# real-stanford/semantic-abstraction

Hardware: AMD Instinct MI355X
Metric: scenes/sec (relevancy+3D-UNet infer), 480x480x16-label x128^3 (higher is better)
Workload: dtype f16 (MFMA operands, fp32 accumulate; UNet hi/lo-split = fp32-equivalent); 1 GPU; end-to-end relevancy->fusion->OVSSC per scene: 480x480 RGB-D, 16 labels, ViT-B/16, 'ours' saliency config (2448 tile forwards), 128^3 voxels, 80000 input points; scene-sharded; arch=ViT-B/16, unet_precision=exact, tile_chunk_streams=1, scenes_per_gpu=26, parallelism=scene-shard x1, mode=throughput

## Files before the change

### semantic-abstraction_amd/csrc/gemm.hip

```cpp
#include "semabs_common.h"
#include <hip/hip_ext.h>
#include <type_traits>
#include <mutex>

#define BK 64
enum { EPI_BIAS_F16 = 0, EPI_BIAS_GELU_F16 = 1, EPI_BIAS_RESID_F32 = 2, EPI_BIAS_F32 = 3, EPI_ROWMAP_ADD_F32 = 4, EPI_MULROW_F16 = 5 };

struct GemmArgs {
    const f16* A; const f16* B; void* C; const float* bias; const float* addend;
    long M; int N, K; long lda; int ldb; long ldc;
    int g_in, g_out, g_off;
    int n_tiles_n; int n_tiles_m; int group_m; int n_blocks;
    int sc_w;
    int reverse;
    f16* ln_xg; const float* ln_gamma; float* ln_part;
    const float* ln_center;
    const float* ln_rowac; const float* ln_colsum;
    f16* lo_out; int lo_cols; long ld_lo;
#ifdef SEMABS_TUNING
    int ablate;
    unsigned long long* trace;
    unsigned long long* ptrace; int ptrace_wg;
#endif
};
#ifdef SEMABS_TUNING
#define GEMM_ABL(bit) ((g.ablate & (bit)) != 0)
#else
#define GEMM_ABL(bit) (false)
#endif

template <int BKT>
__device__ __forceinline__ int swz_off(int row, int chunk) {
    if (BKT == 64) return row * 128 + ((chunk ^ ((row >> 1) & 7)) << 4);
    return row * 64 + ((chunk ^ ((row >> 2) & 3)) << 4);
}

template <int N> __device__ __forceinline__ void wait_vmcnt() { asm volatile("s_waitcnt vmcnt(%0)" ::"n"(N) : "memory"); }

template <int EPI, int BM, int BN, int BKT, int WGM, int WGN, int STAGES>
__global__ __launch_bounds__(64 * WGM * WGN, ((BM / WGM) * (BN / WGN) <= 64 * 64 && WGM * WGN >= 8) ? 4 : 2) void k_gemm_f16(GemmArgs g) {
    constexpr int NW = WGM * WGN;
    constexpr int WTM = BM / WGM, WTN = BN / WGN, TM = WTM / 32, TN = WTN / 32;
    constexpr int ROWB = BKT * 2;
    constexpr int RPP = 1024 / ROWB;
    constexpr int CPR = ROWB / 16;
    constexpr int A_BYTES = BM * ROWB, BUF = (BM + BN) * ROWB;
    constexpr int PPW = (BM + BN) / RPP / NW;
    static_assert((BM + BN) / RPP % NW == 0 && WTN == 64 && WTM % 32 == 0 && STAGES >= 2, "tile / wave layout");
    static_assert(STAGES * BUF >= NW * 8192, "epilogue staging needs 8 KB per wave");
    extern __shared__ __attribute__((aligned(16))) char smem[];
    const int tid = threadIdx.x, lane = tid & 63;
    const int wid = __builtin_amdgcn_readfirstlane(tid >> 6);
    const int wm = wid / WGN, wn = wid % WGN;

    int b = blockIdx.x;
    {
        const int nb = g.n_blocks, q = nb >> 3, r = nb & 7, xcd = b & 7, k = b >> 3;
        b = (xcd < r ? xcd * (q + 1) : r * (q + 1) + (xcd - r) * q) + k;
    }
    int tm, tn;
    {
        const int per_group = g.group_m * g.n_tiles_n, gid = b / per_group, first_m = gid * g.group_m;
        const int gsz = (g.n_tiles_m - first_m < g.group_m) ? g.n_tiles_m - first_m : g.group_m;
        const int r = b - gid * per_group;
        tm = first_m + r % gsz; tn = r / gsz;
    }
    const long m0 = (long)tm * BM;
    const int n0 = tn * BN;

    const f16* src[PPW];
// ... 70 lines not shown
    __builtin_amdgcn_s_barrier();

    if (GEMM_ABL(8) && acc[0][0][0] != 12345.678f) return;
    float* st = reinterpret_cast<float*>(smem + wid * 8192);
    const int cchunk = lane & 15;
    const int ncol = n0 + wn * WTN + cchunk * 4;
    float4 bv = make_float4(0.f, 0.f, 0.f, 0.f);
    if (g.bias) bv = *reinterpret_cast<const float4*>(g.bias + ncol);
#pragma unroll
    for (int i = 0; i < TM; ++i) {
#pragma unroll
        for (int j = 0; j < 2; ++j)
#pragma unroll
            for (int r = 0; r < 16; ++r) {
                int row = (r & 3) + 8 * (r >> 2) + 4 * (lane >> 5);
                st[row * 64 + j * 32 + (lane & 31)] = acc[i][j][r];
            }
        __builtin_amdgcn_s_waitcnt(0xc07f);
        __builtin_amdgcn_wave_barrier();
        if (EPI == EPI_BIAS_F16 || EPI == EPI_BIAS_GELU_F16) {
            const int c8 = lane & 7;
            const int ncol8 = n0 + wn * WTN + c8 * 8;
            float4 b0 = make_float4(0.f, 0.f, 0.f, 0.f), b1 = b0;
            if (g.bias) { b0 = *reinterpret_cast<const float4*>(g.bias + ncol8); b1 = *reinterpret_cast<const float4*>(g.bias + ncol8 + 4); }
#pragma unroll
            for (int it = 0; it < 4; ++it) {
                const int row = it * 8 + (lane >> 3);
                const long m = m0 + wm * WTM + i * 32 + row;
                if (m >= g.M) continue;
                const float4 v0 = *reinterpret_cast<const float4*>(st + row * 64 + c8 * 8);
                const float4 v1 = *reinterpret_cast<const float4*>(st + row * 64 + c8 * 8 + 4);
                float v[8] = {v0.x + b0.x, v0.y + b0.y, v0.z + b0.z, v0.w + b0.w, v1.x + b1.x, v1.y + b1.y, v1.z + b1.z, v1.w + b1.w};
                f16x8 h;
#pragma unroll
                for (int e = 0; e < 8; ++e) {
                    if (EPI == EPI_BIAS_GELU_F16) v[e] = v[e] * __builtin_amdgcn_rcpf(1.f + __expf(-1.702f * v[e]));
                    h[e] = (f16)v[e];
                }
                if (GEMM_ABL(16) && v[0] != 12345.678f) continue;
                *reinterpret_cast<f16x8*>(reinterpret_cast<f16*>(g.C) + m * g.ldc + ncol8) = h;
            }
        } else {
#pragma unroll 4
        for (int it = 0; it < 8; ++it) {
            int row = it * 4 + (lane >> 4);
            long m = m0 + wm * WTM + i * 32 + row;
            if (m >= g.M) continue;
            float4 v = *reinterpret_cast<const float4*>(st + row * 64 + cchunk * 4);
            v.x += bv.x; v.y += bv.y; v.z += bv.z; v.w += bv.w;
            if (GEMM_ABL(16) && v.x != 12345.678f) continue;
            if (EPI == EPI_BIAS_RESID_F32) {
                float4* p = reinterpret_cast<float4*>(reinterpret_cast<float*>(g.C) + m * g.ldc + ncol);
                float4 o = *p;
                o.x += v.x; o.y += v.y; o.z += v.z; o.w += v.w;
                *p = o;
            } else if (EPI == EPI_BIAS_F32) {
                *reinterpret_cast<float4*>(reinterpret_cast<float*>(g.C) + m * g.ldc + ncol) = v;
            } else {
                long grp = m / g.g_in; int within = (int)(m - grp * g.g_in);
                long orow = grp * g.g_out + g.g_off + within;
                if (g.addend) {
                    float4 a = *reinterpret_cast<const float4*>(g.addend + (long)(g.g_off + within) * g.N + ncol);
                    v.x += a.x; v.y += a.y; v.z += a.z; v.w += a.w;
                }
                *reinterpret_cast<float4*>(reinterpret_cast<float*>(g.C) + orow * g.ldc + ncol) = v;
            }
        }
        }
        __builtin_amdgcn_wave_barrier();
    }
}
// ... 193 lines not shown
            __builtin_amdgcn_sched_barrier(0);
            asm volatile("s_nop 7\n\ts_nop 7" ::: "memory");
            __builtin_amdgcn_sched_barrier(0);
        };
        constexpr int ROWB = OUT16 ? 64 : 128;
        constexpr int LPR = ROWB / 16;
        constexpr int RPI = 64 / LPR;
        constexpr int NIT = 64 / RPI;
        constexpr int PASSB = 64 * ROWB;
        char* const ep = smem + wid * 16384;
        float bia[2][8];
#pragma unroll
        for (int hb = 0; hb < 2; ++hb) {
            const int ncol = n0 + hb * 128 + wc * 32 + kg * 8;
#pragma unroll
            for (int e = 0; e < 8; ++e) bia[hb][e] = 0.f;
            if (g.bias) {
                const float4 b0 = *reinterpret_cast<const float4*>(g.bias + ncol), b1 = *reinterpret_cast<const float4*>(g.bias + ncol + 4);
                bia[hb][0] = b0.x; bia[hb][1] = b0.y; bia[hb][2] = b0.z; bia[hb][3] = b0.w; bia[hb][4] = b1.x; bia[hb][5] = b1.y; bia[hb][6] = b1.z; bia[hb][7] = b1.w;
            }
        }
        const int wswz = OUT16 ? ((l15 >> 1) & 3) : (l15 & 7);
        auto lds_write = [&](int pass) {
            const int hb = pass >> 1, ha = pass & 1;
            char* buf = ep + (pass & 1) * PASSB;
            f32x4 w[4][OUT16 ? 1 : 2];
#pragma unroll
            for (int i = 0; i < 4; ++i) {
                float v[8];
#pragma unroll
                for (int e = 0; e < 4; ++e) { v[e] = acc[ha][i][hb][0][e] + bia[hb][e]; v[4 + e] = acc[ha][i][hb][1][e] + bia[hb][4 + e]; }
                if constexpr (OUT16) {
                    f16x8 h;
#pragma unroll
                    for (int e = 0; e < 8; ++e) {
                        if (EPI == EPI_BIAS_GELU_F16) v[e] = v[e] * __builtin_amdgcn_rcpf(1.f + __expf(-1.702f * v[e]));
                        h[e] = (f16)v[e];
                    }
                    w[i][0] = __builtin_bit_cast(f32x4, h);
                } else {
                    w[i][0] = f32x4{v[0], v[1], v[2], v[3]};
                    w[i][OUT16 ? 0 : 1] = f32x4{v[4], v[5], v[6], v[7]};
                }
            }
            __builtin_amdgcn_sched_barrier(0);
#pragma unroll
            for (int i = 0; i < 4; ++i) {
                char* row = buf + (i * 16 + l15) * ROWB;
                if constexpr (OUT16) {
                    *reinterpret_cast<f32x4*>(row + ((kg ^ wswz) << 4)) = w[i][0];
                } else {
                    *reinterpret_cast<f32x4*>(row + (((2 * kg) ^ wswz) << 4)) = w[i][0];
                    *reinterpret_cast<f32x4*>(row + (((2 * kg + 1) ^ wswz) << 4)) = w[i][OUT16 ? 0 : 1];
                }
            }
            __builtin_amdgcn_sched_barrier(0);
        };
        const int crow = lane / LPR, cchunk = lane % LPR;
        auto lds_read = [&](int pass, int it) {
            const int row = it * RPI + crow;
            const int rswz = OUT16 ? ((row >> 1) & 3) : (row & 7);
            return *reinterpret_cast<const f32x4*>(ep + (pass & 1) * PASSB + row * ROWB + ((cchunk ^ rswz) << 4));
        };
        const long mw = m0 + wr * 64;
        const unsigned ldcb = (unsigned)g.ldc * ES;
        if constexpr (EPI == EPI_ROWMAP_ADD_F32) {
            const long grp0 = mw / g.g_in; const long orow0 = grp0 * g.g_out + g.g_off + (mw - grp0 * g.g_in);
            const long mlast = g.M - 1; const long grpl = mlast / g.g_in; const long orowl = grpl * g.g_out + g.g_off + (mlast - grpl * g.g_in);
            const __amdgpu_buffer_rsrc_t rC = gemm_rsrc(reinterpret_cast<const float*>(g.C) + orow0 * g.ldc + (n0 + wc * 32),
                                                        (orowl - orow0) * (long)ldcb + (long)(g.N - n0 - wc * 32) * ES);
#pragma unroll
// ... 502 lines not shown
        if (wid == 0 || wid == 4) {
            const int nst = g.K / 64 * 16;
            for (int i = lane; i < nst && i < 1024; i += 64)
                g.ptrace[(wid >> 2) * 1024 + i] = *reinterpret_cast<unsigned long long*>(smem + 2 * BUFSZ + (wid >> 2) * 8192 + i * 8);
        }
    }
#endif
#ifdef SEMABS_TUNING
    if (g.trace) {
        asm volatile("s_waitcnt vmcnt(0)" ::: "memory");
        const unsigned long long t_end = __builtin_amdgcn_s_memrealtime();
        if (tid == 0) {
            unsigned hw, xcc;
            asm volatile("s_getreg_b32 %0, hwreg(HW_REG_HW_ID)" : "=s"(hw));
            asm volatile("s_getreg_b32 %0, hwreg(HW_REG_XCC_ID)" : "=s"(xcc));
            unsigned long long* tr = g.trace + (size_t)vb * 8;
            tr[0] = t_start; tr[1] = t_main; tr[2] = t_end; tr[3] = ((unsigned long long)xcc << 32) | hw; tr[4] = c_start; tr[5] = c_main;
        }
    }
#endif
    if (PERS) {
        __builtin_amdgcn_s_waitcnt(0xc07f);
        __builtin_amdgcn_s_barrier();
    }
    vb += (int)gridDim.x;
    } while (PERS && vb < g.n_blocks);
#undef GABL
#undef GEMM8_SYNC
#undef GEMM8_END
#undef GEMM8_INTERLEAVE
#undef GEMM8_STAMP
}

template <int EPI, bool LNC = false, bool QKLO = false>
__global__ __launch_bounds__(512) void k_gemm8p(GemmArgs g) {
    static_assert(!QKLO || EPI == EPI_BIAS_F16, "the low halves exist for the plain fp16 output only");
    static_assert(EPI == EPI_BIAS_F16 || EPI == EPI_BIAS_GELU_F16 || EPI == EPI_BIAS_RESID_F32, "fp16-output epilogues and the fp32 residual read-modify-write");
    static_assert(!LNC || EPI != EPI_BIAS_RESID_F32, "the LayerNorm consumer has fp16 outputs");
    constexpr bool OUT16 = EPI != EPI_BIAS_RESID_F32;
    constexpr int HT = 16384, OFF_A0 = 0, OFF_B0 = HT, OFF_B1 = 2 * HT, OFF_A1 = 3 * HT, BUFSZ = 4 * HT;
    constexpr int OFF_SCR = 2 * BUFSZ, OFF_BIAS = OFF_SCR + 8 * 2048;
    constexpr int OFF_CS = OFF_BIAS + 2 * 1024, OFF_RA = OFF_CS + 2 * 1024;
    extern __shared__ __attribute__((aligned(16))) char smem[];
    const int tid = threadIdx.x, lane = tid & 63;
    const int wid = __builtin_amdgcn_readfirstlane(tid >> 6);
    const int wr = wid >> 2, wc = wid & 3;
    const int l15 = lane & 15, kg = lane >> 4;
    const bool has_bias = g.bias != nullptr;

    auto tile_of = [&](int vb, long& m0, int& n0) {
        const int b = semabs_xcd_item(vb, g.n_blocks, g.reverse != 0);
        const int per_group = g.group_m * g.n_tiles_n, gid = b / per_group, first_m = gid * g.group_m;
        const int gsz = (g.n_tiles_m - first_m < g.group_m) ? g.n_tiles_m - first_m : g.group_m;
        const int r = b - gid * per_group;
        m0 = (long)(first_m + r % gsz) * 256;
        n0 = (r / gsz) * 256;
    };
    const int srow = tid >> 3, scp = tid & 7;
    const unsigned aoff = (unsigned)(srow * (int)g.lda * 2 + (swzA8(srow, scp) - srow * 128));
    const unsigned boff = (unsigned)(srow * g.ldb * 2 + (swzB8(srow, scp) - srow * 128));
    const unsigned a_half = (unsigned)(128 * (int)g.lda * 2), b_half = (unsigned)(128 * g.ldb * 2);
    const unsigned a_q = (unsigned)(64 * (int)g.lda * 2), b_q = (unsigned)(64 * g.ldb * 2);
    __amdgpu_buffer_rsrc_t rA, rB, rAn, rBn;
    const __amdgpu_buffer_rsrc_t rBias = gemm_rsrc(g.bias, has_bias ? (long)g.N * 4 : 0);
    [[maybe_unused]] const __amdgpu_buffer_rsrc_t rCs = gemm_rsrc(g.ln_colsum, LNC ? (long)g.N * 4 : 0);
    [[maybe_unused]] const __amdgpu_buffer_rsrc_t rRa = gemm_rsrc(g.ln_rowac, LNC ? (g.M * 8 > 0x7fffffffL ? 0x7fffffffL : g.M * 8) : 0);
    auto rsrc_a = [&](long m0) { const long rows = g.M - m0 < 256 ? g.M - m0 : 256; return gemm_rsrc(g.A + m0 * g.lda, ((rows - 1) * g.lda + g.K) * 2); };
    auto rsrc_b = [&](int n0) { return gemm_rsrc(g.B + (long)n0 * g.ldb, (255L * g.ldb + g.K) * 2); };
    auto stage = [&](const int j, const int kt, const bool nx) {
        const bool isa = j == 0 || j == 3, hi = j >= 2;
        char* dst = smem + (kt & 1) * BUFSZ + (j == 0 ? OFF_A0 : (j == 1 ? OFF_B0 : (j == 2 ? OFF_B1 : OFF_A1))) + wid * 1024;
        const unsigned soff = (unsigned)kt * 128 + (hi ? (isa ? a_half : b_half) : 0u);
        const __amdgpu_buffer_rsrc_t r = isa ? (nx ? rAn : rA) : (nx ? rBn : rB);
#ifdef SEMABS_TUNING
        if ((isa && (g.ablate & 64)) || (!isa && (g.ablate & 128))) {
// ... 24 lines not shown
    }
    f32x4 acc[2][4][2][2];
    f16x8 fa[4][2], fa1[4][2], fb[2][2][2], fb0n[2][2];
    auto mma = [&](const int ha, const int hb, const f16x8 (&a)[4][2], const f16x8 (&b)[2][2]) {
#pragma unroll
        for (int kk = 0; kk < 2; ++kk)
#pragma unroll
            for (int i = 0; i < 4; ++i)
#pragma unroll
                for (int j = 0; j < 2; ++j)
                    acc[ha][i][hb][j] = __builtin_amdgcn_mfma_f32_16x16x32_f16(b[j][kk], a[i][kk], acc[ha][i][hb][j], 0, 0, 0);
    };
    typedef const __attribute__((address_space(3))) char* lds_cptr;
    typedef const __attribute__((address_space(3))) f16x8* lds_frag;
    auto pin = [&](int x) { lds_cptr p = (lds_cptr)smem + x; asm volatile("" : "+v"(p)); return p; };
    auto rd_a = [&](f16x8 (&dst)[4][2], lds_cptr r0, lds_cptr r1, const int off) {
#pragma unroll
        for (int i = 0; i < 4; ++i) { dst[i][0] = *(lds_frag)(r0 + (off + i * 2048)); dst[i][1] = *(lds_frag)(r1 + (off + i * 2048)); }
    };
    auto rd_b = [&](f16x8 (&dst)[2][2], lds_cptr r0, lds_cptr r1, const int off) {
#pragma unroll
        for (int j = 0; j < 2; ++j) { dst[j][0] = *(lds_frag)(r0 + (off + j * 512)); dst[j][1] = *(lds_frag)(r1 + (off + j * 512)); }
    };
#define P_INTERLEAVE(nread)                                                      \
    do {                                                                         \
        _Pragma("unroll") for (int q_ = 0; q_ < (nread); ++q_) {                 \
            __builtin_amdgcn_sched_group_barrier(0x008, 1, 0);                   \
            __builtin_amdgcn_sched_group_barrier(0x100, 1, 0);                   \
        }                                                                        \
        __builtin_amdgcn_sched_group_barrier(0x008, 16 - (nread), 0);            \
    } while (0)
    const int nk = g.K / 64;
    constexpr int VM_AFTER_EPI = OUT16 ? 26 : 63;
    bool prev_lo = false;
    auto ktile = [&](auto steady_c, const int t, const int kts, const bool nx, const int st_ph) {
        constexpr bool STEADY = decltype(steady_c)::value;
        const int pb = (t & 1) * BUFSZ, pn = pb ^ BUFSZ;
        const bool pen = t + 2 == nk;
        lds_cptr r0, r1;
#define P_SYNC(k_)                                                               \
    do {                                                                         \
        if (STEADY) { if ((k_) < st_ph) { if (QKLO && prev_lo) wait_vmcnt<VM_AFTER_EPI + 16>(); else wait_vmcnt<VM_AFTER_EPI>(); } else wait_vmcnt<10>(); } \
        else if (pen) wait_vmcnt<8 - 2 * (k_)>();                                \
        else if ((k_) == 0) wait_vmcnt<0>();                                     \
        __builtin_amdgcn_s_waitcnt(0xc07f);                                      \
        __builtin_amdgcn_sched_barrier(0);                                       \
        __builtin_amdgcn_s_setprio(1);                                           \
        __builtin_amdgcn_s_barrier();                                            \
        __builtin_amdgcn_sched_barrier(0);                                       \
    } while (0)
#define P_END()                                                                  \
    do {                                                                         \
        __builtin_amdgcn_sched_barrier(0);                                       \
        __builtin_amdgcn_s_setprio(0);                                           \
        __builtin_amdgcn_s_barrier();                                            \
        __builtin_amdgcn_sched_barrier(0);                                       \
    } while (0)
        if (STEADY) stage(0, kts, nx);
        r0 = pin(offB[0] + pb); r1 = pin(offB[1] + pb);
        P_SYNC(0);
        rd_b(fb[1], r0, r1, OFF_B1); mma(0, 0, fa, fb[0]);
        P_INTERLEAVE(4);
        P_END();
        if (STEADY) stage(1, kts, nx);
        r0 = pin(offA[0] + pb); r1 = pin(offA[1] + pb);
        P_SYNC(1);
        rd_a(fa1, r0, r1, OFF_A1); mma(0, 1, fa, fb[1]);
        P_INTERLEAVE(8);
        P_END();
        if (STEADY) stage(2, kts, nx);
        r0 = pin(offA[0] + pn); r1 = pin(offA[1] + pn);
        P_SYNC(2);
        rd_a(fa, r0, r1, OFF_A0); mma(1, 1, fa1, fb[1]);
        P_INTERLEAVE(8);
        P_END();
        if (STEADY) stage(3, kts, nx);
        r0 = pin(offB[0] + pn); r1 = pin(offB[1] + pn);
        P_SYNC(3);
        rd_b(fb0n, r0, r1, OFF_B0); mma(1, 0, fa1, fb[0]);
        P_INTERLEAVE(4);
        P_END();
        __builtin_amdgcn_s_waitcnt(0xc07f);
#pragma unroll
        for (int j = 0; j < 2; ++j)
#pragma unroll
            for (int kk = 0; kk < 2; ++kk) fb[0][j][kk] = fb0n[j][kk];
    };
    auto epilogue = [&](const long m0, const int n0, const int bpar) {
        int t_ = tid; asm volatile("" : "+v"(t_));
        const int ln = t_ & 63, r15 = ln & 15, q4 = ln >> 4;
        char* const ep = smem + OFF_SCR + wid * 2048;
        f32x4 bia[2][2];
#pragma unroll
        for (int hb = 0; hb < 2; ++hb)
#pragma unroll
            for (int j = 0; j < 2; ++j)
                bia[hb][j] = has_bias ? *reinterpret_cast<const f32x4*>(smem + OFF_BIAS + bpar * 1024 + (hb * 128 + wc * 32 + q4 * 8 + j * 4) * 4) : f32x4{0.f, 0.f, 0.f, 0.f};
        [[maybe_unused]] f32x4 csm[LNC ? 2 : 1][2];
        if constexpr (LNC) {
#pragma unroll
            for (int hb = 0; hb < 2; ++hb)
#pragma unroll
                for (int j = 0; j < 2; ++j)
                    csm[hb][j] = *reinterpret_cast<const f32x4*>(smem + OFF_CS + bpar * 1024 + (hb * 128 + wc * 32 + q4 * 8 + j * 4) * 4);
        }
        const long mw = m0 + wr * 64;
        const long rows = g.M - mw;
        if constexpr (!OUT16) {
            const int wswz8 = r15 & 7;
// ... 47 lines not shown
        [[maybe_unused]] const unsigned ldlob = (unsigned)g.ld_lo * 2u;
        [[maybe_unused]] const __amdgpu_buffer_rsrc_t rLo = gemm_rsrc(reinterpret_cast<const char*>(g.lo_out) + (mw * g.ld_lo + n0 + wc * 32) * 2,
                                                                       (QKLO && tile_lo && rows > 0) ? (rows - 1) * (long)ldlob + (long)(g.lo_cols - n0 - wc * 32) * 2 : 0);
        [[maybe_unused]] const unsigned volo = (unsigned)crow * ldlob + (unsigned)(cchunk * 16);
#pragma unroll
        for (int pass = 0; pass < 4; ++pass) {
            const int hb = pass >> 1, ha = pass & 1;
            [[maybe_unused]] float2 rap[LNC ? 4 : 1];
            if constexpr (LNC) {
#pragma unroll
                for (int i = 0; i < 4; ++i) rap[i] = *reinterpret_cast<const float2*>(smem + OFF_RA + bpar * 2048 + (ha * 128 + wr * 64 + i * 16 + r15) * 8);
            }
#pragma unroll
            for (int hf = 0; hf < 2; ++hf) {
                f32x4 w[2];
                [[maybe_unused]] f32x4 wl[QKLO ? 2 : 1];
#pragma unroll
                for (int il = 0; il < 2; ++il) {
                    const int i = hf * 2 + il;
                    float v[8];
                    if constexpr (LNC) {
                        const float2 ra = rap[i];
#pragma unroll
                        for (int e = 0; e < 4; ++e) {
                            v[e] = acc[ha][i][hb][0][e] * ra.x + (ra.y * csm[hb][0][e] + bia[hb][0][e]);
                            v[4 + e] = acc[ha][i][hb][1][e] * ra.x + (ra.y * csm[hb][1][e] + bia[hb][1][e]);
                        }
                    } else {
#pragma unroll
                        for (int e = 0; e < 4; ++e) { v[e] = acc[ha][i][hb][0][e] + bia[hb][0][e]; v[4 + e] = acc[ha][i][hb][1][e] + bia[hb][1][e]; }
                    }
                    f16x8 h;
                    [[maybe_unused]] f16x8 hl;
#pragma unroll
                    for (int e = 0; e < 8; ++e) {
                        if (EPI == EPI_BIAS_GELU_F16) v[e] = v[e] * __builtin_amdgcn_rcpf(1.f + __expf(-1.702f * v[e]));
                        h[e] = (f16)v[e];
                        if constexpr (QKLO) hl[e] = (f16)(v[e] - (float)h[e]);
                    }
                    w[il] = __builtin_bit_cast(f32x4, h);
                    if constexpr (QKLO) wl[il] = __builtin_bit_cast(f32x4, hl);
                }
                __builtin_amdgcn_sched_barrier(0);
#pragma unroll
                for (int il = 0; il < 2; ++il) *reinterpret_cast<f32x4*>(ep + (il * 16 + r15) * 64 + ((q4 ^ wswz) << 4)) = w[il];
                __builtin_amdgcn_sched_barrier(0);
#pragma unroll
                for (int it = 0; it < 2; ++it) {
                    const int row = it * 16 + crow;
                    const f32x4 v = *reinterpret_cast<const f32x4*>(ep + row * 64 + ((cchunk ^ ((row >> 1) & 3)) << 4));
#ifdef SEMABS_TUNING
                    if (g.ablate & 32) { buf_store4<2>(rC, voff, (unsigned)(ha * 128 + hf * 32 + it * 16) * ldcb + (unsigned)(hb * 128 * 2), v); continue; }
                    if (g.ablate & 256) { buf_store4<17>(rC, voff, (unsigned)(ha * 128 + hf * 32 + it * 16) * ldcb + (unsigned)(hb * 128 * 2), v); continue; }
                    if (g.ablate & 512) { buf_store4<18>(rC, voff, (unsigned)(ha * 128 + hf * 32 + it * 16) * ldcb + (unsigned)(hb * 128 * 2), v); continue; }
                    if (g.ablate & 1024) { buf_store4<1>(rC, voff, (unsigned)(ha * 128 + hf * 32 + it * 16) * ldcb + (unsigned)(hb * 128 * 2), v); continue; }
                    if (g.ablate & 2048) { buf_store4<16>(rC, voff, (unsigned)(ha * 128 + hf * 32 + it * 16) * ldcb + (unsigned)(hb * 128 * 2), v); continue; }
                    if (g.ablate & 4096) { buf_store4<19>(rC, voff, (unsigned)(ha * 128 + hf * 32 + it * 16) * ldcb + (unsigned)(hb * 128 * 2), v); continue; }
#endif
                    buf_store4<0>(rC, voff, (unsigned)(ha * 128 + hf * 32 + it * 16) * ldcb + (unsigned)(hb * 128 * 2), v);
                }
                __builtin_amdgcn_sched_barrier(0);
                asm volatile("s_nop 7\n\ts_nop 7" ::: "memory");
                __builtin_amdgcn_sched_barrier(0);
                if constexpr (QKLO) {
                    if (tile_lo) {
#pragma unroll
                        for (int il = 0; il < 2; ++il) *reinterpret_cast<f32x4*>(ep + (il * 16 + r15) * 64 + ((q4 ^ wswz) << 4)) = wl[il];
                        __builtin_amdgcn_sched_barrier(0);
#pragma unroll
                        for (int it = 0; it < 2; ++it) {
                            const int row = it * 16 + crow;
                            const f32x4 v = *reinterpret_cast<const f32x4*>(ep + row * 64 + ((cchunk ^ ((row >> 1) & 3)) << 4));
                            buf_store4<0>(rLo, volo, (unsigned)(ha * 128 + hf * 32 + it * 16) * ldlob + (unsigned)(hb * 128 * 2), v);
                        }
                        __builtin_amdgcn_sched_barrier(0);
                        asm volatile("s_nop 7\n\ts_nop 7" ::: "memory");
                        __builtin_amdgcn_sched_barrier(0);
                    }
                }
            }
        }
    };

    int vb = blockIdx.x;
    long m0; int n0;
    tile_of(vb, m0, n0);
    rA = rsrc_a(m0); rB = rsrc_b(n0);
    bool first = true;
    int bpar = 0;
    stage_bias(m0, n0, 0);
    stage(0, 0, false); stage(1, 0, false); stage(2, 0, false); stage(3, 0, false); stage(0, 1, false); stage(1, 1, false); stage(2, 1, false); stage(3, 1, false);
    for (;;) {
        const int nvb = vb + (int)gridDim.x;
        const bool has_next = nvb < g.n_blocks;
        long m0n = 0; int n0n = 0;
        if (has_next) { tile_of(nvb, m0n, n0n); rAn = rsrc_a(m0n); rBn = rsrc_b(n0n); } else { rAn = gemm_rsrc(g.A, 0); rBn = gemm_rsrc(g.B, 0); }
#ifdef SEMABS_TUNING
        unsigned long long t_start = 0, t_main = 0, c_start = 0, c_main = 0, t_first = 0;
        if (g.trace) { t_start = __builtin_amdgcn_s_memrealtime(); c_start = __builtin_amdgcn_s_memtime(); }
#endif
        if (first) wait_vmcnt<10>(); else if (QKLO && prev_lo) wait_vmcnt<VM_AFTER_EPI + 16>(); else wait_vmcnt<VM_AFTER_EPI>();
        __builtin_amdgcn_s_barrier();
#ifdef SEMABS_TUNING
        if (g.trace) t_first = __builtin_amdgcn_s_memrealtime();
#endif
#pragma unroll
        for (int a = 0; a < 2; ++a)
#pragma unroll
            for (int i = 0; i < 4; ++i)
#pragma unroll
                for (int c = 0; c < 2; ++c)
#pragma unroll
                    for (int j = 0; j < 2; ++j) acc[a][i][c][j] = f32x4{0.f, 0.f, 0.f, 0.f};
        {
            lds_cptr r0 = pin(offB[0]), r1 = pin(offB[1]);
            rd_b(fb[0], r0, r1, OFF_B0);
            r0 = pin(offA[0]); r1 = pin(offA[1]);
            rd_a(fa, r0, r1, OFF_A0);
        }
        __builtin_amdgcn_s_waitcnt(0xc07f);
        __builtin_amdgcn_s_barrier();
        if (wr == 1) __builtin_amdgcn_s_barrier();
        for (int t = 0; t < nk; ++t) {
            const bool nx = t + 2 >= nk;
            if (has_next && t + 2 == nk) stage_bias(m0n, n0n, bpar ^ 1);
            ktile(std::integral_constant<bool, true>{}, t, nx ? t + 2 - nk : t + 2, nx, first ? 0 : (t == 0 ? 4 : (t == 1 ? 1 : 0)));
        }
        if (wr == 0) __builtin_amdgcn_s_barrier();
#ifdef SEMABS_TUNING
        if (g.trace) { t_main = __builtin_amdgcn_s_memrealtime(); c_main = __builtin_amdgcn_s_memtime(); }
#endif
        epilogue(m0, n0, bpar);
#ifdef SEMABS_TUNING
        if (g.trace && tid == 0) {
            unsigned long long* tr = g.trace + (size_t)vb * 8;
            tr[0] = t_start; tr[1] = t_main; tr[2] = __builtin_amdgcn_s_memrealtime(); tr[3] = 0; tr[4] = c_start; tr[5] = c_main; tr[6] = t_first;
        }
#endif
        if (!has_next) { wait_vmcnt<0>(); break; }
        if constexpr (QKLO) prev_lo = n0 < g.lo_cols;
        vb = nvb; m0 = m0n; n0 = n0n; rA = rAn; rB = rBn; first = false; bpar ^= 1;
    }
#undef P_INTERLEAVE
#undef P_SYNC
#undef P_END
}

static inline int gemm8_group_m(int n_tiles_n) { return n_tiles_n <= 3 ? 2 : (n_tiles_n <= 9 ? 4 : 8); }


template <int EPI>
static int launch_gemm8(GemmArgs g, hipStream_t s, const GemmOpts& o) {
#ifdef SEMABS_TUNING
    constexpr int LDS = 2 * 4 * 16384 + 16384;
#else
    constexpr int LDS = 2 * 4 * 16384;
#endif
    static SemabsLdsAttr attr_pf, attr_nopf;
    semabs_ensure_lds(&k_gemm8<EPI, true>, LDS, attr_pf);
    semabs_ensure_lds(&k_gemm8<EPI, false>, LDS, attr_nopf);
    g.n_tiles_n = g.N / 256;
    const long mt = (g.M + 255) / 256;
    g.n_tiles_m = (int)mt;
    g.group_m = GEMM_GROUP_M > 0 ? GEMM_GROUP_M : gemm8_group_m(g.n_tiles_n);
    g.sc_w = GEMM_SC_W;
    GEMM_TUNE_ARGS(g);
    if (mt * g.n_tiles_n >= (1L << 30)) { semabs_set_error("semabs_gemm_f16: grid too large"); return SEMABS_EINVAL; }
    g.n_blocks = (int)(mt * g.n_tiles_n);
#ifdef SEMABS_TUNING
    if (g_persist) {
        static SemabsLdsAttr attr_p;
        semabs_ensure_lds(&k_gemm8<EPI, true, true>, LDS, attr_p);
        const int ncu = semabs_stream_cus(s);
        gemm_dispatch(k_gemm8<EPI, true, true>, dim3(g.n_blocks < ncu ? g.n_blocks : ncu), dim3(512), LDS, s, g, o);
// ... 1 lines not shown
        return SEMABS_OK;
    }
#endif
#ifdef SEMABS_TUNING
    if constexpr (EPI == EPI_BIAS_F16 || EPI == EPI_BIAS_RESID_F32) {
        if (g_ablate & 31) {
            auto go = [&](auto kern) {
                (void)hipFuncSetAttribute(reinterpret_cast<const void*>(kern), hipFuncAttributeMaxDynamicSharedMemorySize, LDS);
                gemm_dispatch(kern, dim3(g.n_blocks), dim3(512), LDS, s, g, o);
            };
#define GEMM8_ABL_CASE(n) case n: if (o.v2) go(k_gemm8<EPI, true, false, false, true, n>); else go(k_gemm8<EPI, true, false, false, false, n>); break;
            switch (g_ablate & 31) {
                GEMM8_ABL_CASE(8) GEMM8_ABL_CASE(9) GEMM8_ABL_CASE(10) GEMM8_ABL_CASE(11) GEMM8_ABL_CASE(12) GEMM8_ABL_CASE(13) GEMM8_ABL_CASE(15)
                default: semabs_set_error("semabs_gemm_tune: this ablation mask is not instantiated"); return SEMABS_EINVAL;
            }
#undef GEMM8_ABL_CASE
            SEMABS_CHECK_LAUNCH();
            return SEMABS_OK;
        }
    }
#endif
    if constexpr (EPI == EPI_BIAS_RESID_F32) {
        if (g.ln_xg) {
            static SemabsLdsAttr attr_lp;
            semabs_ensure_lds(&k_gemm8<EPI, true, false, false, true, 0, true>, LDS + 16384, attr_lp);
            gemm_dispatch(k_gemm8<EPI, true, false, false, true, 0, true>, dim3(g.n_blocks), dim3(512), LDS + 16384, s, g, o);
            SEMABS_CHECK_LAUNCH();
            return SEMABS_OK;
        }
    }
    if constexpr (EPI == EPI_BIAS_F16 || EPI == EPI_BIAS_GELU_F16) {
        if (g.ln_rowac || g.lo_out) {
            if ((g.K / 64) % 2 != 0) { semabs_set_error("semabs_gemm_f16_ln: the persistent kernel needs an even number of 64-wide K tiles"); return SEMABS_EINVAL; }
            constexpr int LDSC = 2 * 4 * 16384 + 8 * 2048 + 2 * 1024 + 2 * 1024 + 2 * 2048;
            const int ncu = semabs_stream_cus(s);
            const dim3 grid(g.n_blocks < ncu ? g.n_blocks : ncu);
            if constexpr (EPI == EPI_BIAS_F16) {
                if (g.lo_out && g.ln_rowac) {
                    static SemabsLdsAttr a1; semabs_ensure_lds(&k_gemm8p<EPI, true, true>, LDSC, a1);
                    gemm_dispatch(k_gemm8p<EPI, true, true>, grid, dim3(512), LDSC, s, g, o);
                    SEMABS_CHECK_LAUNCH();
                    return SEMABS_OK;
                }
                if (g.lo_out) {
                    static SemabsLdsAttr a2; semabs_ensure_lds(&k_gemm8p<EPI, false, true>, LDSC, a2);
                    gemm_dispatch(k_gemm8p<EPI, false, true>, grid, dim3(512), LDSC, s, g, o);
                    SEMABS_CHECK_LAUNCH();
                    return SEMABS_OK;
                }
            }
            if (g.lo_out) { semabs_set_error("semabs_gemm_f16_ln: low halves exist for epi 0 only"); return SEMABS_EINVAL; }
            static SemabsLdsAttr attr_lc;
            semabs_ensure_lds(&k_gemm8p<EPI, true>, LDSC, attr_lc);
            gemm_dispatch(k_gemm8p<EPI, true>, grid, dim3(512), LDSC, s, g, o);
            SEMABS_CHECK_LAUNCH();
            return SEMABS_OK;
        }
    }
    if (o.ring) {
        static SemabsLdsAttr attr_r;
        semabs_ensure_lds(&k_gemm8<EPI, false, false, true>, LDS, attr_r);
        gemm_dispatch(k_gemm8<EPI, false, false, true>, dim3(g.n_blocks), dim3(512), LDS, s, g, o);
        SEMABS_CHECK_LAUNCH();
        return SEMABS_OK;
    }
    if constexpr (EPI == EPI_BIAS_F16 || EPI == EPI_BIAS_GELU_F16) {
        if (o.v2 && !o.nopers && (g.K / 64) % 2 == 0 && g.sc_w == 0) {
            constexpr int LDSP = 2 * 4 * 16384 + 8 * 2048 + 2 * 1024;
            static SemabsLdsAttr attr_p4;
            semabs_ensure_lds(&k_gemm8p<EPI>, LDSP, attr_p4);
            const int ncu = semabs_stream_cus(s);
            gemm_dispatch(k_gemm8p<EPI>, dim3(g.n_blocks < ncu ? g.n_blocks : ncu), dim3(512), LDSP, s, g, o);
            SEMABS_CHECK_LAUNCH();
            return SEMABS_OK;
        }
    }
    if (o.v2) {
        static SemabsLdsAttr attr_v;
        semabs_ensure_lds(&k_gemm8<EPI, true, false, false, true>, LDS, attr_v);
        gemm_dispatch(k_gemm8<EPI, true, false, false, true>, dim3(g.n_blocks), dim3(512), LDS, s, g, o);
        SEMABS_CHECK_LAUNCH();
        return SEMABS_OK;
    }
    if (GEMM_PREFETCH) gemm_dispatch(k_gemm8<EPI, true>, dim3(g.n_blocks), dim3(512), LDS, s, g, o);
    else gemm_dispatch(k_gemm8<EPI, false>, dim3(g.n_blocks), dim3(512), LDS, s, g, o);
    SEMABS_CHECK_LAUNCH();
    return SEMABS_OK;
}

template <int EPI>
static int launch(const GemmArgs& g, hipStream_t s, const GemmOpts& o) {
    const bool big_ok = g.N % 256 == 0 && g.K >= 128 && g.lda < (1L << 20) && g.ldb < (1 << 20) && g.ldc < (1L << 20);
#ifdef SEMABS_TUNING
    if (g_force_cfg == 3 && g.N % 256 == 0) return launch_cfg<EPI, 256, 256, 32, 4, 4, 4>(g, s, o);
    if (g_force_cfg == 4 && g.N % 256 == 0) return launch_cfg<EPI, 256, 128, 32, 4, 2, 3>(g, s, o);
    if (g_force_cfg == 5 && g.N % 256 == 0) return launch_cfg<EPI, 128, 256, 32, 2, 4, 3>(g, s, o);
    if (g_force_cfg == 6) return launch_cfg<EPI, 128, 128, 32, 2, 2, 3>(g, s, o);
    if (g_force_cfg == 7 && g.N % 256 == 0) return launch_cfg<EPI, 256, 128, 32, 2, 2, 3>(g, s, o);
    if (g_force_cfg == 9 && g.N % 256 == 0) return launch_cfg<EPI, 256, 256, 32, 2, 4, 4>(g, s, o);
#endif
    const bool big = o.kernel == 2 ? big_ok : (o.kernel == 1 ? false : (big_ok && g.M >= 2048));
// ... 86 lines not shown
```

Measured before the change: 8.827 scenes/s.

## Roll persistent GEMM epilogue into next tile's K loop and vectorize QuickGELU

In the persistent fp16-output GEMM kernel, the epilogue for each output tile is split into eight half-quadrant pieces. These pieces are interleaved with the first and last K-tile stages of the next tile, so epilogue stores and conversions overlap with MFMA work instead of running as a separate serialized phase. To support this, the bias/colsum/rowac staging ring grows from two to three buffers, wait counts are retuned per phase, and accumulators are zeroed piecewise. QuickGELU is also rewritten as a packed two-wide helper using exp2 and rcp, which adds register pressure and complexity to the vmcnt bookkeeping.

```diff
diff --git a/semantic-abstraction_amd/csrc/gemm.hip b/semantic-abstraction_amd/csrc/gemm.hip
--- a/semantic-abstraction_amd/csrc/gemm.hip
+++ b/semantic-abstraction_amd/csrc/gemm.hip
@@ -36,6 +36,18 @@
 }
 
 template <int N> __device__ __forceinline__ void wait_vmcnt() { asm volatile("s_waitcnt vmcnt(%0)" ::"n"(N) : "memory"); }
+
+typedef float f32x2 __attribute__((ext_vector_type(2)));
+__device__ __forceinline__ void quickgelu8(float (&v)[8]) {
+#pragma unroll
+    for (int e = 0; e < 8; e += 2) {
+        const f32x2 x = {v[e], v[e + 1]};
+        const f32x2 t = (x * -1.702f) * 0x1.715476p+0f;
+        const f32x2 s = f32x2{__builtin_amdgcn_exp2f(t.x), __builtin_amdgcn_exp2f(t.y)} + 1.f;
+        const f32x2 y = x * f32x2{__builtin_amdgcn_rcpf(s.x), __builtin_amdgcn_rcpf(s.y)};
+        v[e] = y.x; v[e + 1] = y.y;
+    }
+}
 
 template <int EPI, int BM, int BN, int BKT, int WGM, int WGN, int STAGES>
 __global__ __launch_bounds__(64 * WGM * WGN, ((BM / WGM) * (BN / WGN) <= 64 * 64 && WGM * WGN >= 8) ? 4 : 2) void k_gemm_f16(GemmArgs g) {
@@ -172,11 +184,9 @@
                 const float4 v1 = *reinterpret_cast<const float4*>(st + row * 64 + c8 * 8 + 4);
                 float v[8] = {v0.x + b0.x, v0.y + b0.y, v0.z + b0.z, v0.w + b0.w, v1.x + b1.x, v1.y + b1.y, v1.z + b1.z, v1.w + b1.w};
                 f16x8 h;
-#pragma unroll
-                for (int e = 0; e < 8; ++e) {
-                    if (EPI == EPI_BIAS_GELU_F16) v[e] = v[e] * __builtin_amdgcn_rcpf(1.f + __expf(-1.702f * v[e]));
-                    h[e] = (f16)v[e];
-                }
+                if (EPI == EPI_BIAS_GELU_F16) quickgelu8(v);
+#pragma unroll
+                for (int e = 0; e < 8; ++e) h[e] = (f16)v[e];
                 if (GEMM_ABL(16) && v[0] != 12345.678f) continue;
                 *reinterpret_cast<f16x8*>(reinterpret_cast<f16*>(g.C) + m * g.ldc + ncol8) = h;
             }
@@ -436,11 +446,9 @@
                 for (int e = 0; e < 4; ++e) { v[e] = acc[ha][i][hb][0][e] + bia[hb][e]; v[4 + e] = acc[ha][i][hb][1][e] + bia[hb][4 + e]; }
                 if constexpr (OUT16) {
                     f16x8 h;
-#pragma unroll
-                    for (int e = 0; e < 8; ++e) {
-                        if (EPI == EPI_BIAS_GELU_F16) v[e] = v[e] * __builtin_amdgcn_rcpf(1.f + __expf(-1.702f * v[e]));
-                        h[e] = (f16)v[e];
-                    }
+                    if (EPI == EPI_BIAS_GELU_F16) quickgelu8(v);
+#pragma unroll
+                    for (int e = 0; e < 8; ++e) h[e] = (f16)v[e];
                     w[i][0] = __builtin_bit_cast(f32x4, h);
                 } else {
                     w[i][0] = f32x4{v[0], v[1], v[2], v[3]};
@@ -1009,6 +1017,7 @@
 #undef GEMM8_STAMP
 }
 
+constexpr int GEMM8P_NBP = 3;
 template <int EPI, bool LNC = false, bool QKLO = false>
 __global__ __launch_bounds__(512) void k_gemm8p(GemmArgs g) {
     static_assert(!QKLO || EPI == EPI_BIAS_F16, "the low halves exist for the plain fp16 output only");
@@ -1016,8 +1025,10 @@
     static_assert(!LNC || EPI != EPI_BIAS_RESID_F32, "the LayerNorm consumer has fp16 outputs");
     constexpr bool OUT16 = EPI != EPI_BIAS_RESID_F32;
     constexpr int HT = 16384, OFF_A0 = 0, OFF_B0 = HT, OFF_B1 = 2 * HT, OFF_A1 = 3 * HT, BUFSZ = 4 * HT;
+    constexpr bool ROLL = OUT16 && !QKLO;
+    constexpr int NBP = GEMM8P_NBP;
     constexpr int OFF_SCR = 2 * BUFSZ, OFF_BIAS = OFF_SCR + 8 * 2048;
-    constexpr int OFF_CS = OFF_BIAS + 2 * 1024, OFF_RA = OFF_CS + 2 * 1024;
+    constexpr int OFF_CS = OFF_BIAS + NBP * 1024, OFF_RA = OFF_CS + NBP * 1024;
     extern __shared__ __attribute__((aligned(16))) char smem[];
     const int tid = threadIdx.x, lane = tid & 63;
     const int wid = __builtin_amdgcn_readfirstlane(tid >> 6);
@@ -1108,15 +1119,91 @@
     } while (0)
     const int nk = g.K / 64;
     constexpr int VM_AFTER_EPI = OUT16 ? 26 : 63;
+    auto epi_half = [&](const int ha, const int hb, const int hf, const long m0e, const int n0e, const int bpe) {
+        int t_ = tid; asm volatile("" : "+v"(t_));
+        const int ln = t_ & 63, r15 = ln & 15, q4 = ln >> 4;
+        const int wswz = (r15 >> 1) & 3;
+        const int crow = ln >> 2, cchunk = ln & 3;
+        typedef __attribute__((address_space(3))) char* lds_ptr;
+        auto pinw = [&](int x) { lds_ptr p = (lds_ptr)smem + x; asm volatile("" : "+v"(p)); return p; };
+        lds_ptr const ep = pinw(OFF_SCR + wid * 2048 + r15 * 64 + ((q4 ^ wswz) << 4));
+        lds_cptr const er = pin(OFF_SCR + wid * 2048 + crow * 64 + ((cchunk ^ ((crow >> 1) & 3)) << 4));
+        const unsigned ldcb = (unsigned)g.ldc * 2u;
+        const long mw = m0e + wr * 64;
+        const long rows = g.M - mw;
+        const __amdgpu_buffer_rsrc_t rC = gemm_rsrc(reinterpret_cast<const char*>(g.C) + (mw * g.ldc + n0e + wc * 32) * 2,
+                                                    rows > 0 ? (rows - 1) * (long)ldcb + (long)(g.N - n0e - wc * 32) * 2 : 0);
+        const unsigned voff = (unsigned)crow * ldcb + (unsigned)(cchunk * 16);
+        lds_cptr const prow = pin(bpe * 1024 + (wc * 32 + q4 * 8) * 4);
+        [[maybe_unused]] lds_cptr const pra = pin(OFF_RA + bpe * 2048 + (wr * 64 + r15) * 8);
+        f32x4 bia[2];
+        [[maybe_unused]] f32x4 csm[2];
+        [[maybe_unused]] f32x2 rap[2];
+#pragma unroll
+        for (int j = 0; j < 2; ++j) {
+            bia[j] = has_bias ? *(const __attribute__((address_space(3))) f32x4*)(prow + (OFF_BIAS + hb * 512 + j * 16)) : f32x4{0.f, 0.f, 0.f, 0.f};
+            if constexpr (LNC) csm[j] = *(const __attribute__((address_space(3))) f32x4*)(prow + (OFF_CS + hb * 512 + j * 16));
+        }
+        if constexpr (LNC) {
+#pragma unroll
+            for (int il = 0; il < 2; ++il)
+                rap[il] = *(const __attribute__((address_space(3))) f32x2*)(pra + (ha * 128 + (hf * 2 + il) * 16) * 8);
+        }
+        f32x4 w[2];
+#pragma unroll
+        for (int il = 0; il < 2; ++il) {
+            const int i = hf * 2 + il;
+            float v[8];
+            if constexpr (LNC) {
+                const f32x2 ra = rap[il];
+#pragma unroll
+                for (int e = 0; e < 4; ++e) {
+                    v[e] = acc[ha][i][hb][0][e] * ra.x + (ra.y * csm[0][e] + bia[0][e]);
+                    v[4 + e] = acc[ha][i][hb][1][e] * ra.x + (ra.y * csm[1][e] + bia[1][e]);
+                }
+            } else {
+#pragma unroll
+                for (int e = 0; e < 4; ++e) { v[e] = acc[ha][i][hb][0][e] + bia[0][e]; v[4 + e] = acc[ha][i][hb][1][e] + bia[1][e]; }
+            }
+            f16x8 h;
+            if (EPI == EPI_BIAS_GELU_F16) quickgelu8(v);
+#pragma unroll
+            for (int e = 0; e < 8; ++e) h[e] = (f16)v[e];
+            w[il] = __builtin_bit_cast(f32x4, h);
+        }
+        __builtin_amdgcn_sched_barrier(0);
+#pragma unroll
+        for (int il = 0; il < 2; ++il) *(__attribute__((address_space(3))) f32x4*)(ep + il * 1024) = w[il];
+        __builtin_amdgcn_sched_barrier(0);
+#pragma unroll
+        for (int it = 0; it < 2; ++it) {
+            const f32x4 v = *(const __attribute__((address_space(3))) f32x4*)(er + it * 1024);
+            buf_store4<0>(rC, voff, (unsigned)(ha * 128 + hf * 32 + it * 16) * ldcb + (unsigned)(hb * 128 * 2), v);
+        }
+        __builtin_amdgcn_sched_barrier(0);
+        asm volatile("s_nop 7\n\ts_nop 7" ::: "memory");
+        __builtin_amdgcn_sched_barrier(0);
+#pragma unroll
+        for (int il = 0; il < 2; ++il)
+#pragma unroll
+            for (int j = 0; j < 2; ++j) acc[ha][hf * 2 + il][hb][j] = f32x4{0.f, 0.f, 0.f, 0.f};
+    };
     bool prev_lo = false;
-    auto ktile = [&](auto steady_c, const int t, const int kts, const bool nx, const int st_ph) {
+    long e_m0c = 0, e_m0p = 0;
+    int e_n0c = 0, e_n0p = 0, e_bpc = 0, e_bpp = 0;
+#ifdef SEMABS_TUNING
+    unsigned long long t_epi = 0;
+#endif
+    auto ktile = [&](auto steady_c, const int t, const int kts, const bool nx, const int st_ph, const int em) {
         constexpr bool STEADY = decltype(steady_c)::value;
         const int pb = (t & 1) * BUFSZ, pn = pb ^ BUFSZ;
         const bool pen = t + 2 == nk;
+        [[maybe_unused]] const int vm = em >> 2;
         lds_cptr r0, r1;
 #define P_SYNC(k_)                                                               \
     do {                                                                         \
-        if (STEADY) { if ((k_) < st_ph) { if (QKLO && prev_lo) wait_vmcnt<VM_AFTER_EPI + 16>(); else wait_vmcnt<VM_AFTER_EPI>(); } else wait_vmcnt<10>(); } \
+        if (STEADY && ROLL) { if (vm == 0) wait_vmcnt<10>(); else if (vm == 1) wait_vmcnt<10 + 2 * (k_)>(); else if (vm == 2) wait_vmcnt<((k_) == 0 ? 20 : 22)>(); else wait_vmcnt<((k_) == 0 ? 20 : 18 - 2 * (k_))>(); } \
+        else if (STEADY) { if ((k_) < st_ph) { if (QKLO && prev_lo) wait_vmcnt<VM_AFTER_EPI + 16>(); else wait_vmcnt<VM_AFTER_EPI>(); } else wait_vmcnt<10>(); } \
         else if (pen) wait_vmcnt<8 - 2 * (k_)>();                                \
         else if ((k_) == 0) wait_vmcnt<0>();                                     \
         __builtin_amdgcn_s_waitcnt(0xc07f);                                      \
@@ -1133,24 +1220,36 @@
         __builtin_amdgcn_sched_barrier(0);                                       \
     } while (0)
         if (STEADY) stage(0, kts, nx);
+        if constexpr (ROLL) { if (em & 2) { epi_half(0, 1, 1, e_m0p, e_n0p, e_bpp); epi_half(1, 1, 0, e_m0p, e_n0p, e_bpp); } }
         r0 = pin(offB[0] + pb); r1 = pin(offB[1] + pb);
         P_SYNC(0);
         rd_b(fb[1], r0, r1, OFF_B1); mma(0, 0, fa, fb[0]);
         P_INTERLEAVE(4);
         P_END();
         if (STEADY) stage(1, kts, nx);
+        if constexpr (ROLL) { if (em & 1) epi_half(0, 0, 0, e_m0c, e_n0c, e_bpc); else if (em & 2) epi_half(1, 1, 1, e_m0p, e_n0p, e_bpp); }
         r0 = pin(offA[0] + pb); r1 = pin(offA[1] + pb);
         P_SYNC(1);
         rd_a(fa1, r0, r1, OFF_A1); mma(0, 1, fa, fb[1]);
         P_INTERLEAVE(8);
         P_END();
         if (STEADY) stage(2, kts, nx);
+        if constexpr (ROLL) { if (em & 1) epi_half(0, 0, 1, e_m0c, e_n0c, e_bpc); else if (em & 2) epi_half(1, 0, 0, e_m0p, e_n0p, e_bpp); }
         r0 = pin(offA[0] + pn); r1 = pin(offA[1] + pn);
         P_SYNC(2);
         rd_a(fa, r0, r1, OFF_A0); mma(1, 1, fa1, fb[1]);
         P_INTERLEAVE(8);
         P_END();
         if (STEADY) stage(3, kts, nx);
+        if constexpr (ROLL) {
+            if (em & 1) epi_half(0, 1, 0, e_m0c, e_n0c, e_bpc);
+            else if (em & 2) {
+                epi_half(1, 0, 1, e_m0p, e_n0p, e_bpp);
+#ifdef SEMABS_TUNING
+                if (g.trace) t_epi = __builtin_amdgcn_s_memrealtime();
+#endif
+            }
+        }
         r0 = pin(offB[0] + pn); r1 = pin(offB[1] + pn);
         P_SYNC(3);
         rd_b(fb0n, r0, r1, OFF_B0); mma(1, 0, fa1, fb[0]);
@@ -1264,9 +1363,9 @@
                     }
                     f16x8 h;
                     [[maybe_unused]] f16x8 hl;
+                    if (EPI == EPI_BIAS_GELU_F16) quickgelu8(v);
 #pragma unroll
                     for (int e = 0; e < 8; ++e) {
-                        if (EPI == EPI_BIAS_GELU_F16) v[e] = v[e] * __builtin_amdgcn_rcpf(1.f + __expf(-1.702f * v[e]));
                         h[e] = (f16)v[e];
                         if constexpr (QKLO) hl[e] = (f16)(v[e] - (float)h[e]);
                     }
@@ -1321,6 +1420,7 @@
     bool first = true;
     int bpar = 0;
     stage_bias(m0, n0, 0);
+    e_m0c = m0; e_n0c = n0;
     stage(0, 0, false); stage(1, 0, false); stage(2, 0, false); stage(3, 0, false); stage(0, 1, false); stage(1, 1, false); stage(2, 1, false); stage(3, 1, false);
     for (;;) {
         const int nvb = vb + (int)gridDim.x;
@@ -1331,19 +1431,21 @@
         unsigned long long t_start = 0, t_main = 0, c_start = 0, c_main = 0, t_first = 0;
         if (g.trace) { t_start = __builtin_amdgcn_s_memrealtime(); c_start = __builtin_amdgcn_s_memtime(); }
 #endif
-        if (first) wait_vmcnt<10>(); else if (QKLO && prev_lo) wait_vmcnt<VM_AFTER_EPI + 16>(); else wait_vmcnt<VM_AFTER_EPI>();
+        if (first) wait_vmcnt<10>(); else if (ROLL) wait_vmcnt<16>(); else if (QKLO && prev_lo) wait_vmcnt<VM_AFTER_EPI + 16>(); else wait_vmcnt<VM_AFTER_EPI>();
         __builtin_amdgcn_s_barrier();
 #ifdef SEMABS_TUNING
         if (g.trace) t_first = __builtin_amdgcn_s_memrealtime();
 #endif
-#pragma unroll
-        for (int a = 0; a < 2; ++a)
-#pragma unroll
-            for (int i = 0; i < 4; ++i)
-#pragma unroll
-                for (int c = 0; c < 2; ++c)
-#pragma unroll
-                    for (int j = 0; j < 2; ++j) acc[a][i][c][j] = f32x4{0.f, 0.f, 0.f, 0.f};
+        if (first || !ROLL) {
+#pragma unroll
+            for (int a = 0; a < 2; ++a)
+#pragma unroll
+                for (int i = 0; i < 4; ++i)
+#pragma unroll
+                    for (int c = 0; c < 2; ++c)
+#pragma unroll
+                        for (int j = 0; j < 2; ++j) acc[a][i][c][j] = f32x4{0.f, 0.f, 0.f, 0.f};
+        }
         {
             lds_cptr r0 = pin(offB[0]), r1 = pin(offB[1]);
             rd_b(fb[0], r0, r1, OFF_B0);
@@ -1355,23 +1457,33 @@
         if (wr == 1) __builtin_amdgcn_s_barrier();
         for (int t = 0; t < nk; ++t) {
             const bool nx = t + 2 >= nk;
-            if (has_next && t + 2 == nk) stage_bias(m0n, n0n, bpar ^ 1);
-            ktile(std::integral_constant<bool, true>{}, t, nx ? t + 2 - nk : t + 2, nx, first ? 0 : (t == 0 ? 4 : (t == 1 ? 1 : 0)));
+            if (has_next && t + 2 == nk) stage_bias(m0n, n0n, bpar + 1 == NBP ? 0 : bpar + 1);
+            int em = (t + 1 == nk ? 1 : 0) | (t == 0 && !first ? 2 : 0);
+            em |= (em & 2 ? 2 : (em & 1 ? 1 : (t == 1 && !first ? 3 : 0))) << 2;
+            em = __builtin_amdgcn_readfirstlane(em); asm volatile("" : "+s"(em));
+            ktile(std::integral_constant<bool, true>{}, t, nx ? t + 2 - nk : t + 2, nx, first ? 0 : (t == 0 ? 4 : (t == 1 ? 1 : 0)), em);
         }
         if (wr == 0) __builtin_amdgcn_s_barrier();
 #ifdef SEMABS_TUNING
         if (g.trace) { t_main = __builtin_amdgcn_s_memrealtime(); c_main = __builtin_amdgcn_s_memtime(); }
 #endif
-        epilogue(m0, n0, bpar);
+        if constexpr (!ROLL) epilogue(m0, n0, bpar);
+        else if (!has_next) {
+            epi_half(0, 1, 1, m0, n0, bpar); epi_half(1, 1, 0, m0, n0, bpar); epi_half(1, 1, 1, m0, n0, bpar);
+            epi_half(1, 0, 0, m0, n0, bpar); epi_half(1, 0, 1, m0, n0, bpar);
+        }
 #ifdef SEMABS_TUNING
         if (g.trace && tid == 0) {
             unsigned long long* tr = g.trace + (size_t)vb * 8;
             tr[0] = t_start; tr[1] = t_main; tr[2] = __builtin_amdgcn_s_memrealtime(); tr[3] = 0; tr[4] = c_start; tr[5] = c_main; tr[6] = t_first;
+            if (ROLL && !first) (g.trace + (size_t)(vb - (int)gridDim.x) * 8)[2] = t_epi;
         }
 #endif
         if (!has_next) { wait_vmcnt<0>(); break; }
         if constexpr (QKLO) prev_lo = n0 < g.lo_cols;
-        vb = nvb; m0 = m0n; n0 = n0n; rA = rAn; rB = rBn; first = false; bpar ^= 1;
+        e_m0p = m0; e_n0p = n0; e_bpp = bpar;
+        vb = nvb; m0 = m0n; n0 = n0n; rA = rAn; rB = rBn; first = false; bpar = bpar + 1 == NBP ? 0 : bpar + 1;
+        e_m0c = m0; e_n0c = n0; e_bpc = bpar;
     }
 #undef P_INTERLEAVE
 #undef P_SYNC
@@ -1439,7 +1551,7 @@
     if constexpr (EPI == EPI_BIAS_F16 || EPI == EPI_BIAS_GELU_F16) {
         if (g.ln_rowac || g.lo_out) {
             if ((g.K / 64) % 2 != 0) { semabs_set_error("semabs_gemm_f16_ln: the persistent kernel needs an even number of 64-wide K tiles"); return SEMABS_EINVAL; }
-            constexpr int LDSC = 2 * 4 * 16384 + 8 * 2048 + 2 * 1024 + 2 * 1024 + 2 * 2048;
+            constexpr int LDSC = 2 * 4 * 16384 + 8 * 2048 + GEMM8P_NBP * (1024 + 1024 + 2048);
             const int ncu = semabs_stream_cus(s);
             const dim3 grid(g.n_blocks < ncu ? g.n_blocks : ncu);
             if constexpr (EPI == EPI_BIAS_F16) {
@@ -1473,7 +1585,7 @@
     }
     if constexpr (EPI == EPI_BIAS_F16 || EPI == EPI_BIAS_GELU_F16) {
         if (o.v2 && !o.nopers && (g.K / 64) % 2 == 0 && g.sc_w == 0) {
-            constexpr int LDSP = 2 * 4 * 16384 + 8 * 2048 + 2 * 1024;
+            constexpr int LDSP = 2 * 4 * 16384 + 8 * 2048 + GEMM8P_NBP * 1024;
             static SemabsLdsAttr attr_p4;
             semabs_ensure_lds(&k_gemm8p<EPI>, LDSP, attr_p4);
             const int ncu = semabs_stream_cus(s);
```

Result: slower. 7.932 scenes/s (-10.1%).
